# NVIDIA-Genomics-Research/DL4VC

Hardware: AMD Instinct MI355X
Metric: candidate-variants/sec (DAN fwd, 64 reads x 201 bp) (higher is better)
Workload: dtype f32

## Files before the change

### dl4vc_amd/csrc/dan_device.h

```cpp
#pragma once
#include "dan_kernels.h"

namespace dan {

typedef float v4f __attribute__((ext_vector_type(4)));

__device__ __forceinline__ v4f mfma16(float a, float b, v4f c) {
    return __builtin_amdgcn_mfma_f32_16x16x4f32(a, b, c, 0, 0, 0);
}

__device__ __forceinline__ v4f splat(float x) { return (v4f){x, x, x, x}; }

typedef const __attribute__((address_space(1))) v4f* gv4f_ptr;

__device__ __forceinline__ float relu1(float v) { return __builtin_amdgcn_fmed3f(v, 0.f, __builtin_inff()); }

__device__ __forceinline__ void gemm_tile(v4f (&acc)[NT], const v4f (&a)[NT], v4f& b, const float* next) {
#pragma unroll
    for (int s = 0; s < 4; ++s)
#pragma unroll
        for (int n = 0; n < NT; ++n) acc[n] = mfma16(a[n][s], b[s], acc[n]);
    b = *(const v4f*)next;
}

// ... 23 lines not shown
#pragma unroll
        for (int n = 0; n < NT; ++n) a_nxt[n] = wl[(size_t)nx * (KGC * 64) + n * 64];
        int tn = t, gn = g + 1;
        if (gn == kg) { gn = 0; ++tn; }
        if (it + 1 == total) { tn = t; gn = g; }
        const float* xn = xrow + (t0 + tn * dil) * LDS_S + gn * 16;
#pragma unroll
        for (int m = 0; m < MTW - 1; ++m) gemm_tile(acc[m], a, b[m], xn + m * 16 * LDS_S);
        __builtin_amdgcn_sched_group_barrier(0x020, NT, 0);
#pragma unroll
        for (int m = 0; m < MTW - 1; ++m) {
            __builtin_amdgcn_sched_group_barrier(0x008, 4 * NT, 0);
            __builtin_amdgcn_sched_group_barrier(0x100, 1, 0);
        }
        if (full) gemm_tile(acc[MTW - 1], a, b[MTW - 1], xn + (MTW - 1) * 16 * LDS_S);
        if constexpr (JOIN_WAIT) {
            asm volatile("s_nop 7");
            __builtin_amdgcn_sched_barrier(0);
        }
        t = tn; g = gn;
    }
}

template <int NW, bool RANGE = false, int TILES = MT>
__device__ __forceinline__ void bottleneck(const float* xs, const v4f (&wf)[KGC], const float* bbot, float* hrow, int L,
                                           int wave, int lane, int p_lo = 0) {
    constexpr int PSTEP = NW / 2;
    constexpr int NBT = (TILES + PSTEP - 1) / PSTEP;
    lane = (int)__builtin_amdgcn_mbcnt_hi(~0u, __builtin_amdgcn_mbcnt_lo(~0u, 0u));
    asm volatile("" : "+v"(lane));
    const int pos = lane & 15, kk = lane >> 4;
    const int n = wave & 1, p0 = wave >> 1;
    const float* xrow = xs + (HALO + pos) * LDS_S + kk * 4;
    int roff[NBT];
#pragma unroll
    for (int i = 0; i < NBT; ++i) roff[i] = min(p0 + PSTEP * i, TILES - 1) * 16 * LDS_S;
    v4f acc[NBT], b[NBT];
    {
        const v4f bias = *(const v4f*)(bbot + n * 16 + kk * 4);
#pragma unroll
        for (int i = 0; i < NBT; ++i) acc[i] = bias;
    }
#pragma unroll
    for (int i = 0; i < NBT; ++i) b[i] = *(const v4f*)(xrow + roff[i]);
#pragma unroll
    for (int g = 0; g < KGC; ++g) {
        const int gn = (g + 1 < KGC) ? g + 1 : g;
#pragma unroll
        for (int i = 0; i < NBT; ++i) {
#pragma unroll
            for (int s = 0; s < 4; ++s) acc[i] = mfma16(wf[g][s], b[i][s], acc[i]);
            b[i] = *(const v4f*)(xrow + roff[i] + gn * 16);
        }
// ... 166 lines not shown
```

### dl4vc_amd/csrc/dan_kernels.hip

```cpp
#include "dan_device.h"
#include "dan_reduce.h"

namespace dan {

#ifdef DAN_STAMPS
__device__ unsigned long long* g_stamps;
constexpr int NSTAMP = 64;
#define STAMP(k)                                                                                      \
    do {                                                                                              \
        __builtin_amdgcn_sched_barrier(0);                                                            \
        unsigned long long t_ = __builtin_amdgcn_s_memtime();                                         \
        __builtin_amdgcn_s_waitcnt(0xC07F);                                                           \
        if (lane == 0 && (k) < NSTAMP) g_stamps[((size_t)stamp_row * NWAVE + wave) * NSTAMP + (k)] = t_; \
        __builtin_amdgcn_sched_barrier(0);                                                            \
    } while (0)
#else
#define STAMP(k) do {} while (0)
#endif

static_assert((HALO + WHB + 4 * (4 * MW - 1) + 1 + 4 + 1) * LDS_S <= LDS_ROWS * LDS_S + MAX_LAYERS * CST_FLOATS, "wino reads stay inside LDS");
static_assert(WHB + 4 * (4 * MW - 1) + 3 >= MPOS - 1 && 4 * (4 * MW - 1) + 3 >= WHB - 1, "wino tiling covers the read");
static_assert(HALO + MPOS_SHORT + 15 + 2 < LDS_ROWS && MPOS_SHORT + 16 <= MPOS, "the remainder tile's taps stay inside the image");
static_assert(WHB_SHORT + 4 * (4 * MW_SHORT - 1) + 3 >= MPOS_SHORT - 1 && 4 * (4 * MW_SHORT - 1) + 3 >= WHB_SHORT - 1 && WHB_SHORT % 4 == 2,
              "short wino tiling covers its unit");
// ... 22 lines not shown
            if constexpr (REM) {
                if (m + 1 == TW) {
#pragma unroll
                    for (int s = 0; s < 4; ++s) racc = mfma16(a[s], rb[s], racc);
                }
            }
            __builtin_amdgcn_s_setprio(0);
#pragma unroll
            for (int o = 0; o < 2; ++o) b[m][o] = *(const v4f*)(xrow + (4 * m + 2 * o) * LDS_S + gn * 16);
            if constexpr (REM) {
                if (m + 1 == TW) rb = *(const v4f*)(xr + gn * 16);
            }
        }
    }
}

template <bool WINO, bool PERSIST, bool SPLIT, int TW = MW, bool FOLD = false, bool REM = false>
__global__ __launch_bounds__(SEG_THREADS, NWAVE / 4) void segment_kernel(SegmentArgs a_by_value) {
    static_assert(!FOLD || (PERSIST && !SPLIT), "the site-owning form is a persistent one-unit form");
    static_assert(TW == MW ? !(SPLIT && WINO) : (WINO && TW == MW_SHORT), "six tiles per lane: Winograd forms only, and the split one always");
    static_assert(!REM || (WINO && !SPLIT && TW == MW_SHORT), "the remainder tile [190, 206): beside six Winograd tiles of a one-unit read");
    constexpr int TILES = (SPLIT && WINO) ? (MPOS_SHORT + 15) / 16 : MT;
    constexpr bool W43 = WINO && !SPLIT && TW == MW_SHORT;
    __shared__ __attribute__((aligned(16))) float lds[LDS_ROWS * LDS_S + MAX_LAYERS * CST_FLOATS];
    float* const xs = lds;
    float* const cst = lds + LDS_ROWS * LDS_S;
    typedef const __attribute__((address_space(4))) SegmentArgs* kernarg_ptr;
    constexpr int UNITS = SPLIT ? 2 : 1;
    const int n_work = FOLD ? a_by_value.n_sites : (a_by_value.work_count ? *a_by_value.work_count : a_by_value.n_rows) * UNITS;
    const int per = FOLD ? a_by_value.xcd_sites : a_by_value.work_count ? (n_work + 7) >> 3 : a_by_value.xcd_rows * UNITS;
    const int xcd = blockIdx.x & 7;
    int j = blockIdx.x >> 3;
    int wk = xcd * per + j;
    if (j >= per || wk >= n_work) return;
    [[maybe_unused]] int fold_r = 0;
next_row:
    {
    kernarg_ptr ap = (kernarg_ptr)__builtin_amdgcn_kernarg_segment_ptr();
    if (PERSIST) asm volatile("" : "+s"(ap));
    auto args = [&]() -> decltype(auto) { if constexpr (PERSIST) return (*ap); else return (a_by_value); };
    const auto& a = args();
    [[maybe_unused]] const int unit = wk & 1;
    const int L = SPLIT ? (unit ? a.u_len[1] : a.u_len[0]) : a.L;
    const int Lw = SPLIT ? a.Lw : L;
    const int u_off = SPLIT ? (unit ? a.u_off[1] : a.u_off[0]) : 0;
    [[maybe_unused]] const int own_lo = SPLIT ? (unit ? a.own_lo[1] : a.own_lo[0]) : 0;
    [[maybe_unused]] const int own_hi = SPLIT ? (unit ? a.own_hi[1] : a.own_hi[0]) : L;
    [[maybe_unused]] const int stamp_row = FOLD ? wk * a.R + fold_r : wk;
    int tid = threadIdx.x;
    if (PERSIST) asm volatile("" : "+v"(tid));
    const int lane = tid & 63;
    const int wave = __builtin_amdgcn_readfirstlane(tid >> 6);
    const int wrow = SPLIT ? wk >> 1 : wk;
    const int row_index = FOLD ? wk * a.R + fold_r : __builtin_amdgcn_readfirstlane(a.work_count ? a.work[wrow] : wrow);
    const int site = FOLD ? wk : (int)((unsigned)row_index / (unsigned)a.R);
    const int r = FOLD ? fold_r : row_index - site * a.R;
    const size_t read_idx = (size_t)site * a.R + r;
    float* yrow = a.y + (read_idx * (size_t)Lw + u_off) * CPAD;
    float* yout = SPLIT ? a.y_out + (read_idx * (size_t)Lw + u_off) * CPAD : yrow;
    const int pos = lane & 15, kk = lane >> 4;
    const int cq = wave & 3, ph = wave >> 2;
    const int m_base = ph * MTW, cnt = ph ? MT - MTW : MTW;
    int chb[NT];
#pragma unroll
    for (int n = 0; n < NT; ++n) chb[n] = (cq * NT + n) * 16 + kk * 4;

    STAMP(0);
    [[maybe_unused]] const int wP0 = wino_base<TW>(lane);
    [[maybe_unused]] const int wlim = ((lane >> 2) & 1) ? wino_cover(TW) : wino_half_base(TW);
    [[maybe_unused]] const int chw = wave * 16 + kk * 4;
    auto dil_of = [&](int l) { return (l == 0) ? 1 : (l + 1 < a.n_layers ? a.dil_mid : a.dil_final); };
    auto wino_layer = [&](int l) { return WINO && l > 0; };
    constexpr bool CARRY = !(WINO && (PERSIST || W43));
    v4f pc0 = splat(0.f), pc1 = pc0, pc2 = pc0, pc3 = pc0, pn0 = pc0, pn1 = pc0, pn2 = pc0, pn3 = pc0;
    auto first_frags = [&](int l, v4f& f0, v4f& f1, v4f& f2, v4f& f3) {
        const float* blk = a.wl + (size_t)l * LAYER_STRIDE;
        if (wino_layer(l)) {
            gv4f_ptr w0 = (gv4f_ptr)(blk + WW_OFF) + wave * 64 + lane;
            constexpr size_t KS = (size_t)KGC * (KGC * 64);
            f0 = w0[0]; f1 = w0[KS]; f2 = w0[2 * KS]; f3 = w0[3 * KS];
        } else {
            gv4f_ptr w0 = (gv4f_ptr)(blk + W_OFF) + (cq * NT) * 64 + lane;
            f0 = w0[0]; f1 = w0[64];
        }
    };
    const bool l0_lookup = a.l_begin == 0 && a.l0_tab != nullptr && !(a.tap && a.tap_layer == 0) && (a.l_end - a.l_begin) <= L0_MAX_LAYERS;
    float* const tokf = cst + (a.l_end - a.l_begin) * CST_FLOATS;
    if ((!WINO || a.l_begin == 0) && !l0_lookup) first_frags(a.l_begin, pc0, pc1, pc2, pc3);
    auto stage_constants = [&]() {
        for (int i = tid; i < (a.l_end - a.l_begin) * CST_FLOATS; i += SEG_THREADS) {
            const int l = i / CST_FLOATS, j = i - l * CST_FLOATS;
            cst[i] = a.wl[(size_t)(a.l_begin + l) * LAYER_STRIDE + CST_OFF + j];
        }
    };

    if (a.l_begin == 0) {
        if (l0_lookup) {
            for (int i = tid; i < (LDS_ROWS - L) * (LDS_S / 4); i += SEG_THREADS) {
                const int rr = i / (LDS_S / 4), c4 = i - rr * (LDS_S / 4);
                const int row = rr < HALO ? rr : rr + L;
                *(v4f*)(xs + row * LDS_S + c4 * 4) = splat(0.f);
            }
        } else {
            for (int i = tid; i < LDS_ROWS * LDS_S / 4; i += SEG_THREADS) ((v4f*)xs)[i] = splat(0.f);
        }
        stage_constants();
        __syncthreads();
        const size_t rbase = read_idx * (size_t)Lw + u_off, sbase = (size_t)site * Lw + u_off;
        const int p = tid;
        const bool in = p < L;
        int tok = 0, q = 0, st = 0, rf = 0, rm = 0, vm = 0;
        if (in) {
            tok = a.reads[rbase + p]; q = a.qual[rbase + p]; st = a.strand[rbase + p];
            rf = a.ref[sbase + p]; rm = a.ref_mask[sbase + p]; vm = a.var_mask[sbase + p];
        }
        int tok_w = tok, rm_w = rm, vm_w = vm;
        if constexpr (SPLIT) {
            tok_w = rm_w = vm_w = 0;
            if (tid < Lw) { tok_w = a.reads[rbase - u_off + tid]; rm_w = a.ref_mask[sbase - u_off + tid]; vm_w = a.var_mask[sbase - u_off + tid]; }
        }
        const int agree_ref = __syncthreads_and((rm_w == 0) || (tok_w == rm_w));
        const int agree_var = __syncthreads_and((vm_w == 0) || (tok_w == vm_w));
        if (l0_lookup) {
            if (p <= L + 1) {
                const int pc = p - 1;
                int tk = 0, qq = 0, ss = 0, rr = 0, mm = 0, vv = 0;
                const bool inside = pc >= 0 && pc < L;
                if (inside) {
                    tk = a.reads[rbase + pc]; qq = a.qual[rbase + pc]; ss = a.strand[rbase + pc];
                    rr = a.ref[sbase + pc]; mm = a.ref_mask[sbase + pc]; vv = a.var_mask[sbase + pc];
                }
                float* t = tokf + p * L0_TOK;
                const v4f t0 = {__builtin_bit_cast(float, inside ? min(tk, VOCAB - 1) * 10 + min(rr, VOCAB - 1) : 100), (float)qq * 0.01f, (float)ss * 0.5f,
                                (inside && mm != 0) ? 1.f : 0.f};
                const v4f t1 = {(inside && vv != 0 && agree_var) ? 1.f : 0.f, (p == 0 && agree_ref) ? 1.f : 0.f, 0.f, 0.f};
                *(v4f*)t = t0; *(v4f*)(t + 4) = t1;
            }
        } else if (in) {
            float* row = xs + (HALO + p) * LDS_S;
            const float* er = a.emb + min(tok, VOCAB - 1) * EMBED;
            const float* ef = a.emb + min(rf, VOCAB - 1) * EMBED;
            const float* pp = a.pe + (u_off + p) * EMBED;
#pragma unroll
            for (int e = 0; e < EMBED; ++e) {
                const float pv = pp[e];
// ... 10 lines not shown
        const v4f* src = (const v4f*)yrow;
        const v4f* pl = a.pool ? (const v4f*)(a.pool + ((size_t)site * Lw + u_off) * CPAD) : nullptr;
        const int n4 = L * (CPAD / 4);
        constexpr int NP = TILES * 16 * (CPAD / 4) / SEG_THREADS;
        v4f vy[NP], vp[NP];
#pragma unroll
        for (int k = 0; k < NP; ++k) {
            const int i = tid + k * SEG_THREADS;
            vy[k] = (i < n4) ? src[i] : splat(0.f);
        }
        if (pl) {
#pragma unroll
            for (int k = 0; k < NP; ++k) {
                const int i = tid + k * SEG_THREADS;
                vp[k] = (i < n4) ? pl[i] : splat(0.f);
            }
        } else {
#pragma unroll
            for (int k = 0; k < NP; ++k) vp[k] = splat(0.f);
        }
        for (int i = tid; i < (LDS_ROWS - L) * (LDS_S / 4); i += SEG_THREADS) {
            const int rr = i / (LDS_S / 4), c4 = i - rr * (LDS_S / 4);
            const int row = rr < HALO ? rr : rr + L;
            *(v4f*)(xs + row * LDS_S + c4 * 4) = splat(0.f);
        }
        stage_constants();
#pragma unroll
        for (int k = 0; k < NP; ++k) {
            const int i = tid + k * SEG_THREADS;
            if (i < n4) *(v4f*)(xs + (HALO + (i >> 5)) * LDS_S + (i & 31) * 4) = vy[k] + vp[k];
        }
        if (WINO && CARRY) first_frags(a.l_begin, pc0, pc1, pc2, pc3);
    }
    __syncthreads();
    STAMP(1);
    if (a.tap && a.tap_layer == 0 && a.l_begin == 0) copy_out(xs, a.tap + (read_idx * (size_t)Lw + u_off) * CPAD, own_lo, own_hi, tid);

    v4f wbot[KGC];
    auto layer_tail = [&](int l, const float* lc, bool late_prefetch) {
        [[maybe_unused]] const int sb = 2 + (l - a.l_begin) * 8;
        __syncthreads();
        STAMP(sb + 6);
        if (a.tap && a.tap_layer == l + 1) {
            int t = tid;
            asm volatile("" : "+v"(t));
            copy_out(xs, a.tap + (read_idx * (size_t)Lw + u_off) * CPAD, own_lo, own_hi, t);
        }
        if (WINO && CARRY && late_prefetch && l + 1 < a.l_end) first_frags(l + 1, pn0, pn1, pn2, pn3);
        if (!(FOLD && WINO) && a.has_hw && !(WINO && l + 1 < a.l_end) && !(FOLD && l + 1 == a.l_end))
            bottleneck<NWAVE, SPLIT, TILES>(xs, wbot, lc + CST_BBOT, a.h + (size_t)l * a.h_layer_stride + (read_idx * (size_t)Lw + u_off) * HPAD,
                                     own_hi, wave, lane, own_lo);
        STAMP(sb + 7);
        if (CARRY) { pc0 = pn0; pc1 = pn1; pc2 = pn2; pc3 = pn3; }
    };

    auto direct_layer = [&](int l) {
        const float* wblk = a.wl + (size_t)l * LAYER_STRIDE;
        const float* lc = cst + (l - a.l_begin) * CST_FLOATS;
        const bool residual = (a.res_mask >> l) & 1u;
        const int kg = (l == 0) ? KG0 : KGC;
        const int dil = dil_of(l);
        gv4f_ptr w_conv = (gv4f_ptr)(wblk + W_OFF) + (cq * NT) * 64 + lane;
        gv4f_ptr w_res = (gv4f_ptr)(wblk + WRES_OFF) + (cq * NT) * 64 + lane;
        gv4f_ptr w_bot = (gv4f_ptr)(wblk + WBOT_OFF) + lane;
        [[maybe_unused]] const int sb = 2 + (l - a.l_begin) * 8;
        if (!WINO && l + 1 < a.l_end) first_frags(l + 1, pn0, pn1, pn2, pn3);
        const bool from_global = (l == a.l_begin) && (a.l_begin != 0) && (a.pool != nullptr);
        v4f pre_res[NT];
#pragma unroll
        for (int n = 0; n < NT; ++n) pre_res[n] = residual ? w_res[n * 64] : splat(0.f);
        static_assert(NT == 2, "two direct-form fragments are carried");
        const v4f pre_dir[NT] = {pc0, pc1};

        v4f acc[MTW][NT];
        {
            v4f bias[NT];
#pragma unroll
            for (int n = 0; n < NT; ++n) bias[n] = *(const v4f*)(lc + CST_BIAS + chb[n]);
#pragma unroll
            for (int m = 0; m < MTW; ++m)
#pragma unroll
                for (int n = 0; n < NT; ++n) acc[m][n] = bias[n];
        }
        STAMP(sb + 0);
        conv_gemm<W43>(acc, xs, w_conv, pre_dir, kg, 3, dil, lane, m_base, cnt);
        STAMP(sb + 1);
        const bool bot_here = a.has_hw && !(WINO && l + 1 < a.l_end);
        if (bot_here && !residual) {
#pragma unroll
            for (int g = 0; g < KGC; ++g) wbot[g] = w_bot[(g * 2 + (wave & 1)) * 64];
        }
        {
            v4f sc[NT], sh[NT];
#pragma unroll
            for (int n = 0; n < NT; ++n) { sc[n] = *(const v4f*)(lc + CST_SCALE + chb[n]); sh[n] = *(const v4f*)(lc + CST_SHIFT + chb[n]); }
#pragma unroll
            for (int m = 0; m < MTW; ++m) {
                const bool live = ((m_base + m) * 16 + pos) < L;
#pragma unroll
                for (int n = 0; n < NT; ++n) {
                    v4f v = acc[m][n];
#pragma unroll
                    for (int j = 0; j < 4; ++j) v[j] = live ? relu1(v[j]) * sc[n][j] + sh[n][j] : 0.f;
                    acc[m][n] = v;
                }
            }
        }
        STAMP(sb + 2);
        __syncthreads();
// ... 11 lines not shown
                            v4f* cell = (v4f*)(xs + (HALO + (m_base + m) * 16 + pos) * LDS_S + chb[n]);
                            const v4f old = *cell;
                            *cell = acc[m][n];
                            acc[m][n] = old + bres[n];
                        }
                    }
                }
            } else {
#pragma unroll
                for (int m = 0; m < MTW; ++m) {
                    const int p = (m_base + m) * 16 + pos;
                    if (m < cnt) {
#pragma unroll
                        for (int n = 0; n < NT; ++n) {
                            const v4f old = (p < L) ? *(const v4f*)(yrow + (size_t)p * CPAD + chb[n]) : splat(0.f);
                            *(v4f*)(xs + (HALO + p) * LDS_S + chb[n]) = acc[m][n];
                            acc[m][n] = old + bres[n];
                        }
                    }
                }
            }
            __syncthreads();
            STAMP(sb + 4);
            conv_gemm(acc, xs, w_res, pre_res, KGC, 1, 0, lane, m_base, cnt);
            STAMP(sb + 5);
            if (bot_here) {
#pragma unroll
                for (int g = 0; g < KGC; ++g) wbot[g] = w_bot[(g * 2 + (wave & 1)) * 64];
            }
            __syncthreads();
#pragma unroll
            for (int m = 0; m < MTW; ++m) {
                const int p = (m_base + m) * 16 + pos;
                if (m < cnt) {
#pragma unroll
                    for (int n = 0; n < NT; ++n) *(v4f*)(xs + (HALO + p) * LDS_S + chb[n]) = (p < L) ? acc[m][n] : splat(0.f);
                }
            }
        } else {
#pragma unroll
            for (int m = 0; m < MTW; ++m) {
                if (m < cnt) {
#pragma unroll
                    for (int n = 0; n < NT; ++n)
                        *(v4f*)(xs + (HALO + (m_base + m) * 16 + pos) * LDS_S + chb[n]) = acc[m][n];
                }
            }
        }
        layer_tail(l, lc, true);
    };

    [[maybe_unused]] auto wino_layer_body = [&](int l) {
        if constexpr (WINO) {
        const float* wblk = a.wl + (size_t)l * LAYER_STRIDE;
        const float* lc = cst + (l - a.l_begin) * CST_FLOATS;
        const bool residual = (a.res_mask >> l) & 1u;
        gv4f_ptr w_bot = (gv4f_ptr)(wblk + WBOT_OFF) + lane;
        [[maybe_unused]] const int sb = 2 + (l - a.l_begin) * 8;
        const bool from_global = (l == a.l_begin) && (a.l_begin != 0) && (a.pool != nullptr);
        gv4f_ptr w_w = (gv4f_ptr)(wblk + WW_OFF) + wave * 64 + lane;
        gv4f_ptr w_r1 = (gv4f_ptr)(wblk + WRES_OFF) + wave * 64 + lane;
        float* xw = xs + (HALO + wP0) * LDS_S;
        v4f out[TW][2], pre_r1;
        [[maybe_unused]] v4f rout = splat(0.f);
        [[maybe_unused]] int rp = MPOS_SHORT + pos;
        int wp = wP0;
        float* xq;
        {
            constexpr int NTL = W43 ? MW43 : TW, NCP = W43 ? 6 : 4;
            v4f acc[NTL][NCP];
            const v4f bias = *(const v4f*)(lc + CST_BIAS + chw);
#pragma unroll
            for (int m = 0; m < NTL; ++m)
#pragma unroll
                for (int k = 0; k < NCP; ++k) acc[m][k] = (k == 1) ? bias : splat(0.f);
            if constexpr (REM) rout = bias;
            STAMP(sb + 0);
            if constexpr (W43) {
                gv4f_ptr w0 = (gv4f_ptr)(wblk + W43_OFF) + wave * 64 + lane;
                constexpr size_t KS = (size_t)KGC * (KGC * 64);
                const v4f pre_w[6] = {w0[0], w0[KS], w0[2 * KS], w0[3 * KS], w0[4 * KS], w0[5 * KS]};
                conv_gemm_wino43<REM>(acc, xw - 2 * LDS_S + kk * 4, (gv4f_ptr)(wblk + W43_OFF) + wave * 64, (unsigned)lane * 16u, pre_w, rout,
                                      xs + (HALO + rp - 2) * LDS_S + kk * 4, (gv4f_ptr)(wblk + W_OFF) + wave * 64);
            } else if constexpr (CARRY) {
                const v4f pre_w[4] = {pc0, pc1, pc2, pc3};
                conv_gemm_wino(acc, xw - 2 * LDS_S + kk * 4, w_w, pre_w);
            } else {
                gv4f_ptr w0 = w_w;
                const v4f pre_w[4] = {w0[0], w0[(size_t)KGC * (KGC * 64)], w0[(size_t)2 * KGC * (KGC * 64)], w0[(size_t)3 * KGC * (KGC * 64)]};
                conv_gemm_wino(acc, xw - 2 * LDS_S + kk * 4, w_w, pre_w);
            }
            STAMP(sb + 1);
            asm volatile("" : "+v"(wp));
            if constexpr (REM) asm volatile("" : "+v"(rp));
            xq = xs + (HALO + wp) * LDS_S;
            const v4f sc = *(const v4f*)(lc + CST_SCALE + chw), sh = *(const v4f*)(lc + CST_SHIFT + chw);
            const v2f sc_lo = {sc[0], sc[1]}, sc_hi = {sc[2], sc[3]}, sh_lo = {sh[0], sh[1]}, sh_hi = {sh[2], sh[3]};
            auto half = [](v4f v, int h) { return (v2f){v[2 * h], v[2 * h + 1]}; };
            v2f neg1 = {-1.f, -1.f};
            asm volatile("" : "+v"(neg1));
            auto act = [](v2f y, v2f s, v2f t) {
                const v2f r = {relu1(y[0]), relu1(y[1])};
                return __builtin_elementwise_fma(r, s, t);
            };
            if constexpr (W43) {
                v2f c2 = {2.f, 2.f}, c4 = {4.f, 4.f}, c8 = {8.f, 8.f};
                asm volatile("" : "+v"(c2), "+v"(c4), "+v"(c8));
#pragma unroll
                for (int m = 0; m < MW43; ++m) {
                    v2f y[4][2];
#pragma unroll
                    for (int h = 0; h < 2; ++h) {
                        const v2f M0 = half(acc[m][0], h), M1 = half(acc[m][1], h), M2 = half(acc[m][2], h), M3 = half(acc[m][3], h), M4 = half(acc[m][4], h),
                                  M5 = half(acc[m][5], h);
                        const v2f s1 = M1 + M2, d1 = __builtin_elementwise_fma(M2, neg1, M1), s2 = M3 + M4, d2 = __builtin_elementwise_fma(M4, neg1, M3);
                        y[0][h] = M0 + s1 + s2;
                        y[1][h] = __builtin_elementwise_fma(d2, c2, d1);
                        y[2][h] = __builtin_elementwise_fma(s2, c4, s1);
                        y[3][h] = __builtin_elementwise_fma(d2, c8, d1) + M5;
                    }
#pragma unroll
                    for (int o = 0; o < 4; ++o) {
                        const v2f lo = act(y[o][0], sc_lo, sh_lo), hi = act(y[o][1], sc_hi, sh_hi);
                        out[2 * m + (o >> 1)][o & 1] = (v4f){lo[0], lo[1], hi[0], hi[1]};
                    }
                }
            } else {
#pragma unroll
                for (int m = 0; m < TW; ++m) {
                    const v2f y0l = half(acc[m][0], 0) + half(acc[m][1], 0) + half(acc[m][2], 0), y0h = half(acc[m][0], 1) + half(acc[m][1], 1) + half(acc[m][2], 1);
                    const v2f y1l = __builtin_elementwise_fma(half(acc[m][3], 0), neg1, __builtin_elementwise_fma(half(acc[m][2], 0), neg1, half(acc[m][1], 0)));
                    const v2f y1h = __builtin_elementwise_fma(half(acc[m][3], 1), neg1, __builtin_elementwise_fma(half(acc[m][2], 1), neg1, half(acc[m][1], 1)));
                    const v2f o0l = act(y0l, sc_lo, sh_lo), o0h = act(y0h, sc_hi, sh_hi), o1l = act(y1l, sc_lo, sh_lo), o1h = act(y1h, sc_hi, sh_hi);
                    out[m][0] = (v4f){o0l[0], o0l[1], o0h[0], o0h[1]};
                    out[m][1] = (v4f){o1l[0], o1l[1], o1h[0], o1h[1]};
                }
            }
            if constexpr (REM) {
                const v2f rl = act(half(rout, 0), sc_lo, sh_lo), rh = act(half(rout, 1), sc_hi, sh_hi);
                rout = (v4f){rl[0], rl[1], rh[0], rh[1]};
            }
        }
        [[maybe_unused]] float* const rcell = xs + (HALO + rp) * LDS_S + chw;
        int wl = min(wlim, L);
        asm volatile("" : "+v"(wl));
        __builtin_amdgcn_sched_barrier(0);
        pre_r1 = residual ? w_r1[0] : splat(0.f);
        if (CARRY && !residual && l + 1 < a.l_end) first_frags(l + 1, pn0, pn1, pn2, pn3);
        constexpr bool SEED_EARLY = W43;
        [[maybe_unused]] v4f old[TW][2];
        [[maybe_unused]] v4f rold;
        if (SEED_EARLY && residual && !from_global) {
#pragma unroll
            for (int m = 0; m < TW; ++m)
#pragma unroll
                for (int o = 0; o < 2; ++o) {
                    const int p = wp + 4 * m + 2 * o;
                    if (p < wl) old[m][o] = *(const v4f*)(xq + (4 * m + 2 * o) * LDS_S + chw);
                }
            if constexpr (REM) {
                if (rp < L) rold = *(const v4f*)rcell;
            }
        }
        if (a.has_hw && l > a.l_begin && wave < NWAVE / 2) {
            gv4f_ptr w_bp = (gv4f_ptr)(wblk - LAYER_STRIDE + WBOT_OFF) + lane;
#pragma unroll
            for (int g = 0; g < KGC; ++g) wbot[g] = w_bp[(g * 2 + (wave & 1)) * 64];
            bottleneck<NWAVE / 2, SPLIT, TILES>(xs, wbot, lc - CST_FLOATS + CST_BBOT,
                                         a.h + (size_t)(l - 1) * a.h_layer_stride + (read_idx * (size_t)Lw + u_off) * HPAD, own_hi, wave, lane, own_lo);
        }
        const bool bot_here = a.has_hw && !(l + 1 < a.l_end);
        if (bot_here && !residual) {
#pragma unroll
            for (int g = 0; g < KGC; ++g) wbot[g] = w_bot[(g * 2 + (wave & 1)) * 64];
        }
        STAMP(sb + 2);
        __syncthreads();
        STAMP(sb + 3);
        if (residual) {
            const v4f bres = *(const v4f*)(lc + CST_BRES + chw);
            if (from_global) {
#pragma unroll
                for (int m = 0; m < TW; ++m)
#pragma unroll
                    for (int o = 0; o < 2; ++o) {
                        const int p = wp + 4 * m + 2 * o;
                        if (p < wl) {
                            const v4f old = *(const v4f*)((const char*)yrow + (unsigned)(p * CPAD + chw) * 4u);
                            *(v4f*)(xq + (4 * m + 2 * o) * LDS_S + chw) = out[m][o];
                            out[m][o] = old + bres;
                        }
// ... 10 lines not shown
                for (int m = 0; m < TW; ++m)
#pragma unroll
                    for (int o = 0; o < 2; ++o) {
                        const int p = wp + 4 * m + 2 * o;
                        if (p < wl) {
                            v4f* cell = (v4f*)(xq + (4 * m + 2 * o) * LDS_S + chw);
                            if constexpr (!SEED_EARLY) old[m][o] = *cell;
                            *cell = out[m][o];
                            out[m][o] = old[m][o] + bres;
                        }
                    }
                if constexpr (REM) {
                    if (rp < L) {
                        if constexpr (!SEED_EARLY) rold = *(const v4f*)rcell;
                        *(v4f*)rcell = rout;
                        rout = rold + bres;
                    }
                }
            }
            __syncthreads();
            STAMP(sb + 4);
            gemm1x1_wino<TW, REM>(out, xq + kk * 4, w_r1, pre_r1, rout, xs + (HALO + rp) * LDS_S + kk * 4);
            STAMP(sb + 5);
            if (CARRY && l + 1 < a.l_end) first_frags(l + 1, pn0, pn1, pn2, pn3);
            if (bot_here) {
#pragma unroll
                for (int g = 0; g < KGC; ++g) wbot[g] = w_bot[(g * 2 + (wave & 1)) * 64];
            }
            __syncthreads();
#pragma unroll
            for (int m = 0; m < TW; ++m)
#pragma unroll
                for (int o = 0; o < 2; ++o) {
                    const int p = wp + 4 * m + 2 * o;
                    if (p < wl) *(v4f*)(xq + (4 * m + 2 * o) * LDS_S + chw) = out[m][o];
                }
            if constexpr (REM) {
                if (rp < L) *(v4f*)rcell = rout;
            }
        } else {
#pragma unroll
            for (int m = 0; m < TW; ++m)
#pragma unroll
                for (int o = 0; o < 2; ++o) {
                    const int p = wp + 4 * m + 2 * o;
                    if (p < wl) *(v4f*)(xq + (4 * m + 2 * o) * LDS_S + chw) = out[m][o];
                }
            if constexpr (REM) {
                if (rp < L) *(v4f*)rcell = rout;
            }
        }
        layer_tail(l, lc, false);
        }
    };

    auto lookup_layer0 = [&]() {
        const float* lc = cst;
        [[maybe_unused]] const int sb = 2;
        if (!WINO && 1 < a.l_end) first_frags(1, pn0, pn1, pn2, pn3);
        STAMP(sb + 0);
        const int c4 = tid & 31, pr = tid >> 5;
        const v4f bias = *(const v4f*)(lc + CST_BIAS + c4 * 4), sc = *(const v4f*)(lc + CST_SCALE + c4 * 4), sh = *(const v4f*)(lc + CST_SHIFT + c4 * 4);
        v4f wq[3], wst[3], wlen[3], wvar[3];
        {
            const float agree = tokf[5];
#pragma unroll
            for (int t = 0; t < 3; ++t) {
                auto wv = [&](int k) { return *(const v4f*)(a.l0_tab + L0_WSC_OFF + (k * 3 + t) * CPAD + c4 * 4); };
                wq[t] = wv(0); wst[t] = wv(1); wvar[t] = wv(3);
                wlen[t] = wv(4) + agree * wv(2);
            }
        }
        const v4f* tj = (const v4f*)(a.l0_tab + L0_TJ_OFF) + c4;
        const v4f* pe = (const v4f*)(a.l0_tab + L0_PE_OFF) + (size_t)u_off * (CPAD / 4) + c4;
#pragma unroll 4
        for (int k = 0; k < TILES; ++k) {
            const int p = min(pr + 16 * k, L - 1);
            const int var = (p == 0) ? 1 : (p == L - 1) ? 2 : 0;
            const v4f pe0 = pe[((size_t)var * Lw + p) * (CPAD / 4)];
            v4f s0[3], tv[3];
            v2f s1[3];
#pragma unroll
// ... 24 lines not shown
        }
        STAMP(sb + 2);
        const bool bot_here = a.has_hw && !(WINO && 1 < a.l_end);
        if (bot_here) {
            gv4f_ptr w_bot = (gv4f_ptr)(a.wl + WBOT_OFF) + lane;
#pragma unroll
            for (int g = 0; g < KGC; ++g) wbot[g] = w_bot[(g * 2 + (wave & 1)) * 64];
        }
        layer_tail(0, lc, true);
    };

    if constexpr (WINO) {
        int l = a.l_begin;
        if (l == 0) { if (l0_lookup) lookup_layer0(); else direct_layer(0); l = 1; }
        for (; l < a.l_end; ++l) wino_layer_body(l);
    } else {
        int l = a.l_begin;
        if (l == 0 && l0_lookup) { lookup_layer0(); l = 1; }
        for (; l < a.l_end; ++l) direct_layer(l);
    }
    STAMP(62);
    if constexpr (FOLD) {
        const bool fin = a.fold_feat != nullptr;
        if (!fin) copy_out(xs, yout, own_lo, own_hi, tid);
        constexpr int NF = MT * 16 * (CPAD / 4) / SEG_THREADS;
        const int n4 = L * (CPAD / 4);
        v4f* sp = (v4f*)(a.fold_scratch + (size_t)blockIdx.x * (2 * (size_t)n4 * 4));
        int t = tid;
        asm volatile("" : "+v"(t));
        v4f fsum[NF], fmx[NF];
        if (r > 0) {
#pragma unroll
            for (int k = 0; k < NF; ++k) {
                const int i = t + k * SEG_THREADS;
                fsum[k] = (i < n4) ? sp[i] : splat(0.f);
            }
        } else {
#pragma unroll
            for (int k = 0; k < NF; ++k) fsum[k] = splat(0.f);
        }
        if (r > 0 && fin) {
#pragma unroll
            for (int k = 0; k < NF; ++k) {
                const int i = t + k * SEG_THREADS;
                fmx[k] = (i < n4) ? sp[n4 + i] : splat(0.f);
            }
        } else {
#pragma unroll
            for (int k = 0; k < NF; ++k) fmx[k] = splat(0.f);
        }
        STAMP(56);
        if (a.has_hw) {
            const int ll = a.l_end - 1;
            bottleneck<NWAVE, false, TILES>(xs, wbot, cst + (ll - a.l_begin) * CST_FLOATS + CST_BBOT,
                                            a.h + (size_t)ll * a.h_layer_stride + read_idx * (size_t)Lw * HPAD, own_hi, wave, lane, own_lo);
        }
        STAMP(57);
        const bool last_row = r + 1 == a.R;
#pragma unroll
        for (int k = 0; k < NF; ++k) {
            const int i = t + k * SEG_THREADS;
            const v4f v = (i < n4) ? *(const v4f*)(xs + (HALO + (i >> 5)) * LDS_S + (i & 31) * 4) : splat(0.f);
            v4f mx = v;
            if (r > 0) {
#pragma unroll
                for (int jj = 0; jj < 4; ++jj) mx[jj] = fmaxf(fmx[k][jj], v[jj]);
            }
            fmx[k] = mx;
            v4f sum = fsum[k];
            sum += v;
            fsum[k] = (fin && r == 0) ? v : sum;
        }
        if (!last_row) {
#pragma unroll
            for (int k = 0; k < NF; ++k) {
                const int i = t + k * SEG_THREADS;
                if (i < n4) sp[i] = fsum[k];
// ... 11 lines not shown
            const float fR = (float)a.R;
            __syncthreads();
            auto put = [&](const v4f (&src)[NF]) {
#pragma unroll
                for (int k = 0; k < NF; ++k) {
                    const int i = t + k * SEG_THREADS;
                    if (i < n4) *(v4f*)(xs + (HALO + (i >> 5)) * LDS_S + (i & 31) * 4) = src[k];
                }
            };
            if (!fin) {
                put(fsum);
                v4f* pl = (v4f*)(a.fold_pool + (size_t)site * n4 * 4);
#pragma unroll 1
                for (int i = t; i < n4; i += SEG_THREADS)
                    pl[i] = *(const v4f*)(xs + (HALO + (i >> 5)) * LDS_S + (i & 31) * 4) / splat(fR);
            } else {
                float* row = a.fold_feat + (size_t)site * a.fold_feat_stride;
                const int C = a.fold_C;
                put(fmx);
                __syncthreads();
#pragma unroll 1
                for (int c = wave; c < C; c += NWAVE)
#pragma unroll 1
                    for (int p = lane; p < L; p += 64) row[(unsigned)(c * L + p)] = xs[(HALO + p) * LDS_S + c];
                __syncthreads();
                put(fsum);
                __syncthreads();
                row += (size_t)C * L;
#pragma unroll 1
                for (int c = wave; c < C; c += NWAVE)
#pragma unroll 1
                    for (int p = lane; p < L; p += 64) row[(unsigned)(c * L + p)] = xs[(HALO + p) * LDS_S + c] / fR;
            }
        }
    } else {
        copy_out(xs, yout, own_lo, own_hi, tid);
    }
    STAMP(63);
    }
    if constexpr (FOLD) {
        if (++fold_r == a_by_value.R) {
            fold_r = 0;
            j += gridDim.x >> 3;
            wk = xcd * per + j;
        }
        __syncthreads();
        if (j < per && wk < n_work) goto next_row;
    } else if constexpr (PERSIST) {
        j += gridDim.x >> 3;
        wk = xcd * per + j;
        __syncthreads();
        if (j < per && wk < n_work) goto next_row;
    }
}

int segment_fold_workgroups(int n_sites, int max_wgs) {
    const int w = max_wgs & ~7, need = 8 * ((n_sites + 7) / 8);
    return w < need ? w : need;
}

template <bool PERSIST, bool FOLD>
static void launch_one_unit(const SegmentArgs& a, bool six, bool rem, dim3 grid, hipStream_t s) {
    const dim3 blk(SEG_THREADS);
    if (a.wino && rem) hipLaunchKernelGGL((segment_kernel<true, PERSIST, false, MW_SHORT, FOLD, true>), grid, blk, 0, s, a);
    else if (a.wino && six) hipLaunchKernelGGL((segment_kernel<true, PERSIST, false, MW_SHORT, FOLD>), grid, blk, 0, s, a);
    else if (a.wino) hipLaunchKernelGGL((segment_kernel<true, PERSIST, false, MW, FOLD>), grid, blk, 0, s, a);
    else hipLaunchKernelGGL((segment_kernel<false, PERSIST, false, MW, FOLD>), grid, blk, 0, s, a);
}

void launch_segment(const SegmentArgs& a0, int n_sites, int max_wgs, hipStream_t s) {
// ... 362 lines not shown
```

Measured before the change: 15710.

## Rematerialize lane ids and constants in Winograd kernels to cut live VGPRs

For the Winograd persistent and W43 kernel forms, the lane index, derived offsets and small float constants are recomputed on demand through inline asm (mbcnt, v_mov) instead of being held live across the conv GEMMs. The two __syncthreads_and reductions are merged into a single ballot-plus-LDS workgroup AND, and the persistent walk bounds are reloaded from kernarg each iteration. The aim is to lower register pressure and barrier count. In exchange it adds s_nop padding, extra recomputation and more asm barriers that constrain scheduling.

Measured after the change: 16260 (median of 6 runs). 1.03x the previous value.

```diff
diff --git a/dl4vc_amd/csrc/dan_device.h b/dl4vc_amd/csrc/dan_device.h
--- a/dl4vc_amd/csrc/dan_device.h
+++ b/dl4vc_amd/csrc/dan_device.h
@@ -69,13 +69,28 @@
     }
 }
 
-template <int NW, bool RANGE = false, int TILES = MT>
+__device__ __forceinline__ int lane_now() {
+    int l;
+    asm volatile("s_nop 7\n\ts_nop 2\n\tv_mbcnt_lo_u32_b32 %0, -1, 0\n\tv_mbcnt_hi_u32_b32 %0, -1, %0" : "=v"(l));
+    return l;
+}
+__device__ __forceinline__ float vconst_0() { float x; asm volatile("v_mov_b32 %0, 0" : "=v"(x)); return x; }
+__device__ __forceinline__ float vconst_m1() { float x; asm volatile("v_mov_b32 %0, -1.0" : "=v"(x)); return x; }
+__device__ __forceinline__ float vconst_2() { float x; asm volatile("v_mov_b32 %0, 2.0" : "=v"(x)); return x; }
+__device__ __forceinline__ float vconst_4() { float x; asm volatile("v_mov_b32 %0, 4.0" : "=v"(x)); return x; }
+__device__ __forceinline__ float vconst_8() { float x; asm volatile("v_mov_b32 %0, 0x41000000" : "=v"(x)); return x; }
+
+template <int NW, bool RANGE = false, int TILES = MT, bool FRESH = false>
 __device__ __forceinline__ void bottleneck(const float* xs, const v4f (&wf)[KGC], const float* bbot, float* hrow, int L,
                                            int wave, int lane, int p_lo = 0) {
     constexpr int PSTEP = NW / 2;
     constexpr int NBT = (TILES + PSTEP - 1) / PSTEP;
-    lane = (int)__builtin_amdgcn_mbcnt_hi(~0u, __builtin_amdgcn_mbcnt_lo(~0u, 0u));
-    asm volatile("" : "+v"(lane));
+    if constexpr (FRESH) {
+        lane = lane_now();
+    } else {
+        lane = (int)__builtin_amdgcn_mbcnt_hi(~0u, __builtin_amdgcn_mbcnt_lo(~0u, 0u));
+        asm volatile("" : "+v"(lane));
+    }
     const int pos = lane & 15, kk = lane >> 4;
     const int n = wave & 1, p0 = wave >> 1;
     const float* xrow = xs + (HALO + pos) * LDS_S + kk * 4;
diff --git a/dl4vc_amd/csrc/dan_kernels.hip b/dl4vc_amd/csrc/dan_kernels.hip
--- a/dl4vc_amd/csrc/dan_kernels.hip
+++ b/dl4vc_amd/csrc/dan_kernels.hip
@@ -68,18 +68,34 @@
     static_assert(!REM || (WINO && !SPLIT && TW == MW_SHORT), "the remainder tile [190, 206): beside six Winograd tiles of a one-unit read");
     constexpr int TILES = (SPLIT && WINO) ? (MPOS_SHORT + 15) / 16 : MT;
     constexpr bool W43 = WINO && !SPLIT && TW == MW_SHORT;
+    constexpr bool FRESH = WINO && (PERSIST || W43);
     __shared__ __attribute__((aligned(16))) float lds[LDS_ROWS * LDS_S + MAX_LAYERS * CST_FLOATS];
     float* const xs = lds;
     float* const cst = lds + LDS_ROWS * LDS_S;
+    __shared__ int wg_flags[NWAVE];
     typedef const __attribute__((address_space(4))) SegmentArgs* kernarg_ptr;
     constexpr int UNITS = SPLIT ? 2 : 1;
-    const int n_work = FOLD ? a_by_value.n_sites : (a_by_value.work_count ? *a_by_value.work_count : a_by_value.n_rows) * UNITS;
-    const int per = FOLD ? a_by_value.xcd_sites : a_by_value.work_count ? (n_work + 7) >> 3 : a_by_value.xcd_rows * UNITS;
+    auto walk_bounds = [](const auto& arg, int& n, int& per_slice) {
+        n = FOLD ? arg.n_sites : (arg.work_count ? *arg.work_count : arg.n_rows) * UNITS;
+        per_slice = FOLD ? arg.xcd_sites : arg.work_count ? (n + 7) >> 3 : arg.xcd_rows * UNITS;
+    };
+    int n_work_, per_;
+    walk_bounds(a_by_value, n_work_, per_);
+    const int n_work = n_work_;
+    const int per = per_;
     const int xcd = blockIdx.x & 7;
     int j = blockIdx.x >> 3;
     int wk = xcd * per + j;
     if (j >= per || wk >= n_work) return;
     [[maybe_unused]] int fold_r = 0;
+    [[maybe_unused]] int row_stride = 0;
+    if constexpr (PERSIST && WINO && !FOLD) {
+        row_stride = gridDim.x & ~7;
+        asm volatile("" : "+s"(row_stride));
+    }
+    [[maybe_unused]] int walk = blockIdx.x;
+    if constexpr (PERSIST && WINO && !FOLD) asm volatile("" : "+s"(walk));
+    [[maybe_unused]] const int wave_of_wg = __builtin_amdgcn_readfirstlane((int)threadIdx.x >> 6);
 next_row:
     {
     kernarg_ptr ap = (kernarg_ptr)__builtin_amdgcn_kernarg_segment_ptr();
@@ -93,10 +109,17 @@
     [[maybe_unused]] const int own_lo = SPLIT ? (unit ? a.own_lo[1] : a.own_lo[0]) : 0;
     [[maybe_unused]] const int own_hi = SPLIT ? (unit ? a.own_hi[1] : a.own_hi[0]) : L;
     [[maybe_unused]] const int stamp_row = FOLD ? wk * a.R + fold_r : wk;
-    int tid = threadIdx.x;
-    if (PERSIST) asm volatile("" : "+v"(tid));
+    int tid = threadIdx.x, wave = wave_of_wg;
+    if constexpr (FRESH) {
+        if (PERSIST) asm volatile("" : "+s"(wave));
+        tid = (wave << 6) | lane_now();
+    } else {
+        if (PERSIST) asm volatile("" : "+v"(tid));
+        wave = __builtin_amdgcn_readfirstlane(tid >> 6);
+    }
+    auto tid_now = [&]() { return FRESH ? (wave << 6) | lane_now() : tid; };
+    [[maybe_unused]] const int lane_row = tid & 63;
     const int lane = tid & 63;
-    const int wave = __builtin_amdgcn_readfirstlane(tid >> 6);
     const int wrow = SPLIT ? wk >> 1 : wk;
     const int row_index = FOLD ? wk * a.R + fold_r : __builtin_amdgcn_readfirstlane(a.work_count ? a.work[wrow] : wrow);
     const int site = FOLD ? wk : (int)((unsigned)row_index / (unsigned)a.R);
@@ -104,22 +127,14 @@
     const size_t read_idx = (size_t)site * a.R + r;
     float* yrow = a.y + (read_idx * (size_t)Lw + u_off) * CPAD;
     float* yout = SPLIT ? a.y_out + (read_idx * (size_t)Lw + u_off) * CPAD : yrow;
-    const int pos = lane & 15, kk = lane >> 4;
     const int cq = wave & 3, ph = wave >> 2;
     const int m_base = ph * MTW, cnt = ph ? MT - MTW : MTW;
-    int chb[NT];
-#pragma unroll
-    for (int n = 0; n < NT; ++n) chb[n] = (cq * NT + n) * 16 + kk * 4;
-
     STAMP(0);
-    [[maybe_unused]] const int wP0 = wino_base<TW>(lane);
-    [[maybe_unused]] const int wlim = ((lane >> 2) & 1) ? wino_cover(TW) : wino_half_base(TW);
-    [[maybe_unused]] const int chw = wave * 16 + kk * 4;
     auto dil_of = [&](int l) { return (l == 0) ? 1 : (l + 1 < a.n_layers ? a.dil_mid : a.dil_final); };
     auto wino_layer = [&](int l) { return WINO && l > 0; };
     constexpr bool CARRY = !(WINO && (PERSIST || W43));
     v4f pc0 = splat(0.f), pc1 = pc0, pc2 = pc0, pc3 = pc0, pn0 = pc0, pn1 = pc0, pn2 = pc0, pn3 = pc0;
-    auto first_frags = [&](int l, v4f& f0, v4f& f1, v4f& f2, v4f& f3) {
+    auto first_frags = [&](int l, v4f& f0, v4f& f1, v4f& f2, v4f& f3, int lane) {
         const float* blk = a.wl + (size_t)l * LAYER_STRIDE;
         if (wino_layer(l)) {
             gv4f_ptr w0 = (gv4f_ptr)(blk + WW_OFF) + wave * 64 + lane;
@@ -132,7 +147,7 @@
     };
     const bool l0_lookup = a.l_begin == 0 && a.l0_tab != nullptr && !(a.tap && a.tap_layer == 0) && (a.l_end - a.l_begin) <= L0_MAX_LAYERS;
     float* const tokf = cst + (a.l_end - a.l_begin) * CST_FLOATS;
-    if ((!WINO || a.l_begin == 0) && !l0_lookup) first_frags(a.l_begin, pc0, pc1, pc2, pc3);
+    if ((!WINO || a.l_begin == 0) && !l0_lookup) first_frags(a.l_begin, pc0, pc1, pc2, pc3, lane);
     auto stage_constants = [&]() {
         for (int i = tid; i < (a.l_end - a.l_begin) * CST_FLOATS; i += SEG_THREADS) {
             const int l = i / CST_FLOATS, j = i - l * CST_FLOATS;
@@ -140,15 +155,25 @@
         }
     };
 
+    auto workgroup_and2 = [&](bool p0, bool p1) {
+        const int mine = (__ballot(!p0) == 0ull ? 1 : 0) | (__ballot(!p1) == 0ull ? 2 : 0);
+        if (lane == 0) wg_flags[wave] = mine;
+        __syncthreads();
+        int all = 3;
+#pragma unroll
+        for (int w = 0; w < NWAVE; ++w) all &= wg_flags[w];
+        return all;
+    };
+    const v4f zero4 = splat(FRESH ? vconst_0() : 0.f);
     if (a.l_begin == 0) {
         if (l0_lookup) {
             for (int i = tid; i < (LDS_ROWS - L) * (LDS_S / 4); i += SEG_THREADS) {
                 const int rr = i / (LDS_S / 4), c4 = i - rr * (LDS_S / 4);
                 const int row = rr < HALO ? rr : rr + L;
-                *(v4f*)(xs + row * LDS_S + c4 * 4) = splat(0.f);
+                *(v4f*)(xs + row * LDS_S + c4 * 4) = zero4;
             }
         } else {
-            for (int i = tid; i < LDS_ROWS * LDS_S / 4; i += SEG_THREADS) ((v4f*)xs)[i] = splat(0.f);
+            for (int i = tid; i < LDS_ROWS * LDS_S / 4; i += SEG_THREADS) ((v4f*)xs)[i] = zero4;
         }
         stage_constants();
         __syncthreads();
@@ -165,8 +190,14 @@
             tok_w = rm_w = vm_w = 0;
             if (tid < Lw) { tok_w = a.reads[rbase - u_off + tid]; rm_w = a.ref_mask[sbase - u_off + tid]; vm_w = a.var_mask[sbase - u_off + tid]; }
         }
-        const int agree_ref = __syncthreads_and((rm_w == 0) || (tok_w == rm_w));
-        const int agree_var = __syncthreads_and((vm_w == 0) || (tok_w == vm_w));
+        int agree_ref, agree_var;
+        if constexpr (FRESH) {
+            const int agree_both = workgroup_and2((rm_w == 0) || (tok_w == rm_w), (vm_w == 0) || (tok_w == vm_w));
+            agree_ref = agree_both & 1; agree_var = agree_both & 2;
+        } else {
+            agree_ref = __syncthreads_and((rm_w == 0) || (tok_w == rm_w));
+            agree_var = __syncthreads_and((vm_w == 0) || (tok_w == vm_w));
+        }
         if (l0_lookup) {
             if (p <= L + 1) {
                 const int pc = p - 1;
@@ -223,7 +254,7 @@
         for (int i = tid; i < (LDS_ROWS - L) * (LDS_S / 4); i += SEG_THREADS) {
             const int rr = i / (LDS_S / 4), c4 = i - rr * (LDS_S / 4);
             const int row = rr < HALO ? rr : rr + L;
-            *(v4f*)(xs + row * LDS_S + c4 * 4) = splat(0.f);
+            *(v4f*)(xs + row * LDS_S + c4 * 4) = zero4;
         }
         stage_constants();
 #pragma unroll
@@ -231,7 +262,7 @@
             const int i = tid + k * SEG_THREADS;
             if (i < n4) *(v4f*)(xs + (HALO + (i >> 5)) * LDS_S + (i & 31) * 4) = vy[k] + vp[k];
         }
-        if (WINO && CARRY) first_frags(a.l_begin, pc0, pc1, pc2, pc3);
+        if (WINO && CARRY) first_frags(a.l_begin, pc0, pc1, pc2, pc3, lane);
     }
     __syncthreads();
     STAMP(1);
@@ -243,13 +274,13 @@
         __syncthreads();
         STAMP(sb + 6);
         if (a.tap && a.tap_layer == l + 1) {
-            int t = tid;
-            asm volatile("" : "+v"(t));
+            int t = tid_now();
+            if (!FRESH) asm volatile("" : "+v"(t));
             copy_out(xs, a.tap + (read_idx * (size_t)Lw + u_off) * CPAD, own_lo, own_hi, t);
         }
-        if (WINO && CARRY && late_prefetch && l + 1 < a.l_end) first_frags(l + 1, pn0, pn1, pn2, pn3);
+        if (WINO && CARRY && late_prefetch && l + 1 < a.l_end) first_frags(l + 1, pn0, pn1, pn2, pn3, lane);
         if (!(FOLD && WINO) && a.has_hw && !(WINO && l + 1 < a.l_end) && !(FOLD && l + 1 == a.l_end))
-            bottleneck<NWAVE, SPLIT, TILES>(xs, wbot, lc + CST_BBOT, a.h + (size_t)l * a.h_layer_stride + (read_idx * (size_t)Lw + u_off) * HPAD,
+            bottleneck<NWAVE, SPLIT, TILES, FRESH>(xs, wbot, lc + CST_BBOT, a.h + (size_t)l * a.h_layer_stride + (read_idx * (size_t)Lw + u_off) * HPAD,
                                      own_hi, wave, lane, own_lo);
         STAMP(sb + 7);
         if (CARRY) { pc0 = pn0; pc1 = pn1; pc2 = pn2; pc3 = pn3; }
@@ -263,9 +294,18 @@
         const int dil = dil_of(l);
         gv4f_ptr w_conv = (gv4f_ptr)(wblk + W_OFF) + (cq * NT) * 64 + lane;
         gv4f_ptr w_res = (gv4f_ptr)(wblk + WRES_OFF) + (cq * NT) * 64 + lane;
-        gv4f_ptr w_bot = (gv4f_ptr)(wblk + WBOT_OFF) + lane;
+        int ln = lane, pos = lane & 15, chb[NT];
+        auto lane_share = [&](bool fresh) {
+            if (fresh) {
+                if constexpr (!FRESH) return;
+                ln = lane_now(); pos = ln & 15;
+            }
+#pragma unroll
+            for (int n = 0; n < NT; ++n) chb[n] = (cq * NT + n) * 16 + (ln >> 4) * 4;
+        };
+        lane_share(false);
         [[maybe_unused]] const int sb = 2 + (l - a.l_begin) * 8;
-        if (!WINO && l + 1 < a.l_end) first_frags(l + 1, pn0, pn1, pn2, pn3);
+        if (!WINO && l + 1 < a.l_end) first_frags(l + 1, pn0, pn1, pn2, pn3, lane);
         const bool from_global = (l == a.l_begin) && (a.l_begin != 0) && (a.pool != nullptr);
         v4f pre_res[NT];
 #pragma unroll
@@ -284,8 +324,10 @@
                 for (int n = 0; n < NT; ++n) acc[m][n] = bias[n];
         }
         STAMP(sb + 0);
-        conv_gemm<W43>(acc, xs, w_conv, pre_dir, kg, 3, dil, lane, m_base, cnt);
+        conv_gemm<FRESH || W43>(acc, xs, w_conv, pre_dir, kg, 3, dil, lane, m_base, cnt);
         STAMP(sb + 1);
+        lane_share(true);
+        gv4f_ptr w_bot = (gv4f_ptr)(wblk + WBOT_OFF) + ln;
         const bool bot_here = a.has_hw && !(WINO && l + 1 < a.l_end);
         if (bot_here && !residual) {
 #pragma unroll
@@ -343,11 +385,13 @@
             }
             __syncthreads();
             STAMP(sb + 4);
-            conv_gemm(acc, xs, w_res, pre_res, KGC, 1, 0, lane, m_base, cnt);
+            conv_gemm<FRESH>(acc, xs, w_res, pre_res, KGC, 1, 0, lane, m_base, cnt);
             STAMP(sb + 5);
+            lane_share(true);
             if (bot_here) {
-#pragma unroll
-                for (int g = 0; g < KGC; ++g) wbot[g] = w_bot[(g * 2 + (wave & 1)) * 64];
+                gv4f_ptr w_bl = (gv4f_ptr)(wblk + WBOT_OFF) + ln;
+#pragma unroll
+                for (int g = 0; g < KGC; ++g) wbot[g] = w_bl[(g * 2 + (wave & 1)) * 64];
             }
             __syncthreads();
 #pragma unroll
@@ -373,20 +417,40 @@
 
     [[maybe_unused]] auto wino_layer_body = [&](int l) {
         if constexpr (WINO) {
+        if constexpr (FRESH) {
+            __builtin_assume(l > 0);
+#pragma unroll
+            for (int g = 0; g < KGC; ++g) asm volatile("" : "=v"(wbot[g]));
+        }
         const float* wblk = a.wl + (size_t)l * LAYER_STRIDE;
         const float* lc = cst + (l - a.l_begin) * CST_FLOATS;
         const bool residual = (a.res_mask >> l) & 1u;
-        gv4f_ptr w_bot = (gv4f_ptr)(wblk + WBOT_OFF) + lane;
         [[maybe_unused]] const int sb = 2 + (l - a.l_begin) * 8;
         const bool from_global = (l == a.l_begin) && (a.l_begin != 0) && (a.pool != nullptr);
+        int lane = FRESH ? lane_now() : lane_row;
+        int kk = lane >> 4, chw = wave * 16 + kk * 4, wp = wino_base<TW>(lane);
+        [[maybe_unused]] int rp = MPOS_SHORT + (lane & 15);
+        int wl;
+        float* xq;
+        [[maybe_unused]] float* rcell;
+        auto lane_share = [&](bool behind_conv) {
+            if constexpr (FRESH) {
+                lane = lane_now();
+                kk = lane >> 4; chw = wave * 16 + kk * 4; wp = wino_base<TW>(lane);
+                rp = MPOS_SHORT + (lane & 15);
+            } else {
+                if (!behind_conv) return;
+                asm volatile("" : "+v"(wp));
+            }
+            xq = xs + (HALO + wp) * LDS_S;
+            rcell = xs + (HALO + rp) * LDS_S + chw;
+            wl = min(((lane >> 2) & 1) ? wino_cover(TW) : wino_half_base(TW), L);
+            asm volatile("" : "+v"(wl));
+        };
+        float* xw = xs + (HALO + wp) * LDS_S;
         gv4f_ptr w_w = (gv4f_ptr)(wblk + WW_OFF) + wave * 64 + lane;
-        gv4f_ptr w_r1 = (gv4f_ptr)(wblk + WRES_OFF) + wave * 64 + lane;
-        float* xw = xs + (HALO + wP0) * LDS_S;
         v4f out[TW][2], pre_r1;
         [[maybe_unused]] v4f rout = splat(0.f);
-        [[maybe_unused]] int rp = MPOS_SHORT + pos;
-        int wp = wP0;
-        float* xq;
         {
             constexpr int NTL = W43 ? MW43 : TW, NCP = W43 ? 6 : 4;
             v4f acc[NTL][NCP];
@@ -412,23 +476,19 @@
                 conv_gemm_wino(acc, xw - 2 * LDS_S + kk * 4, w_w, pre_w);
             }
             STAMP(sb + 1);
-            asm volatile("" : "+v"(wp));
-            if constexpr (REM) asm volatile("" : "+v"(rp));
-            xq = xs + (HALO + wp) * LDS_S;
+            lane_share(true);
             const v4f sc = *(const v4f*)(lc + CST_SCALE + chw), sh = *(const v4f*)(lc + CST_SHIFT + chw);
             const v2f sc_lo = {sc[0], sc[1]}, sc_hi = {sc[2], sc[3]}, sh_lo = {sh[0], sh[1]}, sh_hi = {sh[2], sh[3]};
             auto half = [](v4f v, int h) { return (v2f){v[2 * h], v[2 * h + 1]}; };
-            v2f neg1 = {-1.f, -1.f};
-            asm volatile("" : "+v"(neg1));
+            auto pair = [](float x) { return (v2f){x, x}; };
             auto act = [](v2f y, v2f s, v2f t) {
                 const v2f r = {relu1(y[0]), relu1(y[1])};
                 return __builtin_elementwise_fma(r, s, t);
             };
             if constexpr (W43) {
-                v2f c2 = {2.f, 2.f}, c4 = {4.f, 4.f}, c8 = {8.f, 8.f};
-                asm volatile("" : "+v"(c2), "+v"(c4), "+v"(c8));
 #pragma unroll
                 for (int m = 0; m < MW43; ++m) {
+                    const v2f neg1 = pair(vconst_m1()), c2 = pair(vconst_2()), c4 = pair(vconst_4()), c8 = pair(vconst_8());
                     v2f y[4][2];
 #pragma unroll
                     for (int h = 0; h < 2; ++h) {
@@ -447,8 +507,11 @@
                     }
                 }
             } else {
+                v2f neg1_row = {-1.f, -1.f};
+                if constexpr (!FRESH) asm volatile("" : "+v"(neg1_row));
 #pragma unroll
                 for (int m = 0; m < TW; ++m) {
+                    const v2f neg1 = FRESH ? pair(vconst_m1()) : neg1_row;
                     const v2f y0l = half(acc[m][0], 0) + half(acc[m][1], 0) + half(acc[m][2], 0), y0h = half(acc[m][0], 1) + half(acc[m][1], 1) + half(acc[m][2], 1);
                     const v2f y1l = __builtin_elementwise_fma(half(acc[m][3], 0), neg1, __builtin_elementwise_fma(half(acc[m][2], 0), neg1, half(acc[m][1], 0)));
                     const v2f y1h = __builtin_elementwise_fma(half(acc[m][3], 1), neg1, __builtin_elementwise_fma(half(acc[m][2], 1), neg1, half(acc[m][1], 1)));
@@ -462,12 +525,11 @@
                 rout = (v4f){rl[0], rl[1], rh[0], rh[1]};
             }
         }
-        [[maybe_unused]] float* const rcell = xs + (HALO + rp) * LDS_S + chw;
-        int wl = min(wlim, L);
-        asm volatile("" : "+v"(wl));
         __builtin_amdgcn_sched_barrier(0);
+        gv4f_ptr w_bot = (gv4f_ptr)(wblk + WBOT_OFF) + lane;
+        gv4f_ptr w_r1 = (gv4f_ptr)(wblk + WRES_OFF) + wave * 64 + lane;
         pre_r1 = residual ? w_r1[0] : splat(0.f);
-        if (CARRY && !residual && l + 1 < a.l_end) first_frags(l + 1, pn0, pn1, pn2, pn3);
+        if (CARRY && !residual && l + 1 < a.l_end) first_frags(l + 1, pn0, pn1, pn2, pn3, lane);
         constexpr bool SEED_EARLY = W43;
         [[maybe_unused]] v4f old[TW][2];
         [[maybe_unused]] v4f rold;
@@ -487,7 +549,7 @@
             gv4f_ptr w_bp = (gv4f_ptr)(wblk - LAYER_STRIDE + WBOT_OFF) + lane;
 #pragma unroll
             for (int g = 0; g < KGC; ++g) wbot[g] = w_bp[(g * 2 + (wave & 1)) * 64];
-            bottleneck<NWAVE / 2, SPLIT, TILES>(xs, wbot, lc - CST_FLOATS + CST_BBOT,
+            bottleneck<NWAVE / 2, SPLIT, TILES, FRESH>(xs, wbot, lc - CST_FLOATS + CST_BBOT,
                                          a.h + (size_t)(l - 1) * a.h_layer_stride + (read_idx * (size_t)Lw + u_off) * HPAD, own_hi, wave, lane, own_lo);
         }
         const bool bot_here = a.has_hw && !(l + 1 < a.l_end);
@@ -544,10 +606,12 @@
             STAMP(sb + 4);
             gemm1x1_wino<TW, REM>(out, xq + kk * 4, w_r1, pre_r1, rout, xs + (HALO + rp) * LDS_S + kk * 4);
             STAMP(sb + 5);
-            if (CARRY && l + 1 < a.l_end) first_frags(l + 1, pn0, pn1, pn2, pn3);
+            lane_share(false);
+            if (CARRY && l + 1 < a.l_end) first_frags(l + 1, pn0, pn1, pn2, pn3, lane);
             if (bot_here) {
-#pragma unroll
-                for (int g = 0; g < KGC; ++g) wbot[g] = w_bot[(g * 2 + (wave & 1)) * 64];
+                gv4f_ptr w_bl = (gv4f_ptr)(wblk + WBOT_OFF) + lane;
+#pragma unroll
+                for (int g = 0; g < KGC; ++g) wbot[g] = w_bl[(g * 2 + (wave & 1)) * 64];
             }
             __syncthreads();
 #pragma unroll
@@ -579,7 +643,7 @@
     auto lookup_layer0 = [&]() {
         const float* lc = cst;
         [[maybe_unused]] const int sb = 2;
-        if (!WINO && 1 < a.l_end) first_frags(1, pn0, pn1, pn2, pn3);
+        if (!WINO && 1 < a.l_end) first_frags(1, pn0, pn1, pn2, pn3, lane);
         STAMP(sb + 0);
         const int c4 = tid & 31, pr = tid >> 5;
         const v4f bias = *(const v4f*)(lc + CST_BIAS + c4 * 4), sc = *(const v4f*)(lc + CST_SCALE + c4 * 4), sh = *(const v4f*)(lc + CST_SHIFT + c4 * 4);
@@ -650,12 +714,11 @@
     STAMP(62);
     if constexpr (FOLD) {
         const bool fin = a.fold_feat != nullptr;
-        if (!fin) copy_out(xs, yout, own_lo, own_hi, tid);
+        if (!fin) copy_out(xs, yout, own_lo, own_hi, tid_now());
         constexpr int NF = MT * 16 * (CPAD / 4) / SEG_THREADS;
         const int n4 = L * (CPAD / 4);
         v4f* sp = (v4f*)(a.fold_scratch + (size_t)blockIdx.x * (2 * (size_t)n4 * 4));
-        int t = tid;
-        asm volatile("" : "+v"(t));
+        const int t = tid_now();
         v4f fsum[NF], fmx[NF];
         if (r > 0) {
 #pragma unroll
@@ -680,7 +743,7 @@
         STAMP(56);
         if (a.has_hw) {
             const int ll = a.l_end - 1;
-            bottleneck<NWAVE, false, TILES>(xs, wbot, cst + (ll - a.l_begin) * CST_FLOATS + CST_BBOT,
+            bottleneck<NWAVE, false, TILES, FRESH>(xs, wbot, cst + (ll - a.l_begin) * CST_FLOATS + CST_BBOT,
                                             a.h + (size_t)ll * a.h_layer_stride + read_idx * (size_t)Lw * HPAD, own_hi, wave, lane, own_lo);
         }
         STAMP(57);
@@ -738,7 +801,7 @@
 #pragma unroll 1
                 for (int c = wave; c < C; c += NWAVE)
 #pragma unroll 1
-                    for (int p = lane; p < L; p += 64) row[(unsigned)(c * L + p)] = xs[(HALO + p) * LDS_S + c];
+                    for (int p = t & 63; p < L; p += 64) row[(unsigned)(c * L + p)] = xs[(HALO + p) * LDS_S + c];
                 __syncthreads();
                 put(fsum);
                 __syncthreads();
@@ -746,11 +809,15 @@
 #pragma unroll 1
                 for (int c = wave; c < C; c += NWAVE)
 #pragma unroll 1
-                    for (int p = lane; p < L; p += 64) row[(unsigned)(c * L + p)] = xs[(HALO + p) * LDS_S + c] / fR;
-            }
-        }
+                    for (int p = t & 63; p < L; p += 64) row[(unsigned)(c * L + p)] = xs[(HALO + p) * LDS_S + c] / fR;
+            }
+        }
+    } else if constexpr (FRESH && PERSIST) {
+        kernarg_ptr q = (kernarg_ptr)__builtin_amdgcn_kernarg_segment_ptr();
+        asm volatile("" : "+s"(q));
+        copy_out(xs, (SPLIT ? q->y_out : q->y) + (read_idx * (size_t)Lw + u_off) * CPAD, own_lo, own_hi, tid_now());
     } else {
-        copy_out(xs, yout, own_lo, own_hi, tid);
+        copy_out(xs, yout, own_lo, own_hi, tid_now());
     }
     STAMP(63);
     }
@@ -762,6 +829,16 @@
         }
         __syncthreads();
         if (j < per && wk < n_work) goto next_row;
+    } else if constexpr (PERSIST && WINO) {
+        walk += row_stride;
+        const int j_again = walk >> 3, xcd_again = walk & 7;
+        kernarg_ptr q = (kernarg_ptr)__builtin_amdgcn_kernarg_segment_ptr();
+        asm volatile("" : "+s"(q));
+        int n_again, per_again;
+        walk_bounds(*q, n_again, per_again);
+        wk = xcd_again * per_again + j_again;
+        __syncthreads();
+        if (j_again < per_again && wk < n_again) goto next_row;
     } else if constexpr (PERSIST) {
         j += gridDim.x >> 3;
         wk = xcd * per + j;
```
